# chinaxuyongtao/x264-vs2008

Hardware: AMD Instinct MI355X
Metric: encoded frames/sec, 1080p, preset=medium's flag set with the encoder's own lookahead and rate control (--crf 23 --b-adapt 1, hex, subme 7 RD, trellis 1, psy-rd, aq-mode 1, CABAC payload on the GPU); 1/2/4/8 MI355X (bit-exact) (higher is better)
Workload: dtype u8

## Files before the change

### x264_vs2008_amd/csrc/me_exact.h

```cpp
#pragma once
#include "device_prims.h"

#define MX_COST_MAX (1 << 28)
#define MX_COST_LDS 256

static __constant__ int c_subpel_iters[10][4] = {{0,0,0,0},{1,1,0,0},{0,1,1,0},{0,2,1,0},{0,2,1,1},{0,2,1,2},{0,0,2,2},{0,0,2,2},{0,0,4,10},{0,0,4,10}};

#define MX_GLB(T_) const __attribute__((address_space(1))) T_ *
#define MX_LDS(T_) const __attribute__((address_space(3))) T_ *
#define MX_UNI(v_) __builtin_amdgcn_readfirstlane(v_)

#define MX_NIB8(a, b, c_, d, e, f, g, h) ((u32)(((a) & 15) | (((b) & 15) << 4) | (((c_) & 15) << 8) | (((d) & 15) << 12) | (((e) & 15) << 16) | \
                                                (((f) & 15) << 20) | (((g) & 15) << 24) | (((u32)(h) & 15u) << 28)))
__device__ __forceinline__ int mx_nib(u32 pk, int i) { return ((int)(pk << (28 - 4 * i))) >> 28; }
#define MX_HEX2_DX MX_NIB8(-1, -2, -1, 1, 2, 1, -1, -2)
#define MX_HEX2_DY MX_NIB8(-2, 0, 2, 2, 0, -2, -2, 0)
#define MX_DIA_DX MX_NIB8(0, 0, -1, 1, 0, 0, 0, 0)
#define MX_DIA_DY MX_NIB8(-1, 1, 0, 0, 0, 0, 0, 0)

__device__ __forceinline__ void load16u(MX_GLB(u8) p, u32 o[4])
{
    const uintptr_t a = (uintptr_t)p;
    const u32 s = (u32)(a & 3);
    MX_GLB(u32) q = (MX_GLB(u32))(a - s);
// ... 707 lines not shown
            bdir = -1;
            for (int i = qpel; i > 0; i--) {
                const int ox = bx, oyy = by;
                odir = bdir;
                const int x = ox + mx_nib(MX_DIA_DX, g16), y = oyy + mx_nib(MX_DIA_DY, g16);
                const int cost = subpel_sum16_lane(c, x, y, satd, o.chroma_me) + c.lane_cost(x, y);
                const u32 key = mx_best_key<4>(cost, (g16 ^ 1) != odir, lane);
                if ((key >> 3) < (u32)bc) { bdir = (int)(key & 7u); MX_TAKE(4, key, bc, x, y, bx, by); }
                if (bx == ox && by == oyy) break;
            }
            if (by > L.smax1) {
                by = L.smax1;
                bc = __builtin_amdgcn_readlane(subpel_sum16_lane(c, bx, by, satd, o.chroma_me), 0) + c.cost(bx, by);
            }
            out_cost_mv = c.cost(bx, by);
        }
        mvx = bx; mvy = by; mcost = bc;
    } else if (mvy > L.smax1) mvy = L.smax1;
#undef INRANGE
    out_mvx = mvx; out_mvy = mvy;
    return mcost;
}

__device__ __forceinline__ int me_refine_qpel16(const MxCtx &c_in, const MeLimits &L_in, const MeOpts &o_in, int cost_in, int &mvx, int &mvy)
{
    MxCtx c = mx_uniform(c_in);
    c.patch_on = false;
    const MeLimits L = mx_uniform(L_in);
    const MeOpts o = mx_uniform(o_in);
    const int lane = c.lane, g16 = lane >> 4;
    const int hpel = c_subpel_iters[o.subme][0], qpel = c_subpel_iters[o.subme][1], satd = o.subme > 1 && !o.sad_only;
    int bx = MX_UNI(mvx), by = MX_UNI(mvy), bc = MX_UNI(cost_in);
    if (c.has_patch) mx_load_patch(c, bx, by);
    if (hpel && o.subme < 3) {
        const int mx = clip3(c.mvpx, L.smin0, L.smax0), my = clip3(c.mvpy, L.smin1, L.smax1);
        if ((mx - bx) | (my - by)) {
            const int cst = __builtin_amdgcn_readlane(sad_qpel16_lane(c, mx, my), 0) + c.cost(mx, my);
            if (cst < bc) { bc = cst; bx = mx; by = my; }
        }
    }
    for (int i = hpel; i > 0; i--) {
        const int ox = bx, oyy = by;
        const int x = ox + 2 * mx_nib(MX_DIA_DX, g16), y = oyy + 2 * mx_nib(MX_DIA_DY, g16);
        const int cost = sad_qpel16_lane(c, x, y) + c.lane_cost(x, y);
        const u32 key = mx_best_key<4>(cost, true, lane);
        MX_TAKE(4, key, bc, x, y, bx, by);
        if (bx == ox && by == oyy) break;
    }
    for (int i = qpel; i > 0; i--) {
        const int ox = bx, oyy = by;
        const int x = ox + mx_nib(MX_DIA_DX, g16), y = oyy + mx_nib(MX_DIA_DY, g16);
        const int cost = subpel_sum16_lane(c, x, y, satd, o.chroma_me) + c.lane_cost(x, y);
        const u32 key = mx_best_key<4>(cost, true, lane);
        MX_TAKE(4, key, bc, x, y, bx, by);
        if (bx == ox && by == oyy) break;
    }
    if (by > L.smax1) {
        by = L.smax1;
        bc = __builtin_amdgcn_readlane(subpel_sum16_lane(c, bx, by, satd, o.chroma_me), 0) + c.cost(bx, by);
    }
    mvx = bx; mvy = by;
    return bc;
}

__device__ __forceinline__ u32 mr_row_min16(u32 v)
{
    v = min(v, (u32)dpp_mov<0x128>((int)v)); v = min(v, (u32)dpp_mov<0x124>((int)v));
    v = min(v, (u32)dpp_mov<0x122>((int)v)); v = min(v, (u32)dpp_mov<0x121>((int)v));
    return v;
}
__device__ __forceinline__ int mr_from(int v, int src) { return __builtin_amdgcn_ds_bpermute(src << 2, v); }
__device__ __forceinline__ MX_GLB(u8) mr_plane(uint64_t plv, int sb, int k)
{
    const u32 lo = (u32)mr_from((int)(u32)plv, sb + k), hi = (u32)mr_from((int)(u32)(plv >> 32), sb + k);
    return (MX_GLB(u8))(((uint64_t)hi << 32) | lo);
}
__device__ __forceinline__ int mr_cost(const MxCtx &c, int qx, int qy, int mvpx, int mvpy)
{
    const int dx = qx - mvpx, dy = qy - mvpy;
    const bool in = c.has_cost_l && (unsigned)(dx + MX_COST_LDS) <= 2u * MX_COST_LDS && (unsigned)(dy + MX_COST_LDS) <= 2u * MX_COST_LDS;
    if (__ballot(!in) == 0) return (int)c.cost_l[dx + MX_COST_LDS] + (int)c.cost_l[dy + MX_COST_LDS];
    return (int)c.cost_g[dx] + (int)c.cost_g[dy];
}
template <int NR> __device__ __forceinline__ int mr_sad_rows(const MxCtx &c, uint64_t plv, int sb, int qx, int qy, int row0)
{
    const int fx = qx & 3, fy = qy & 3, idx = fy * 4 + fx;
    const ptrdiff_t base = (ptrdiff_t)((qy >> 2) + row0) * c.sy + (qx >> 2);
    MX_GLB(u8) pa = mr_plane(plv, sb, c_qpel_a[idx]) + base + (fy == 3) * c.sy;
    MX_GLB(u8) pb = mr_plane(plv, sb, c_qpel_b[idx]) + base + (fx == 3);
    u32 s = 0;
#pragma unroll
    for (int y = 0; y < NR; y++) {
        u32 a0, a1, t;
        load9u(pa + (ptrdiff_t)y * c.sy, a0, a1, t);
        if (idx & 5) { u32 b0, b1; load9u(pb + (ptrdiff_t)y * c.sy, b0, b1, t); a0 = avg4(a0, b0); a1 = avg4(a1, b1); }
        MX_LDS(u32) f = c.fe + c.fe_off + 4 * (row0 + y);
        s = sad4(a0, f[0], s); s = sad4(a1, f[1], s);
    }
    return (int)s;
}
__device__ __forceinline__ int mr_subpel_sum4(const MxCtx &c, uint64_t plv, int sb, int qx, int qy, int satd, int chroma, int u)
{
    int v = 0;
    u32 d[4][4];
    bool have_d = false;
    const int fx = qx & 3, fy = qy & 3, idx = fy * 4 + fx;
    MX_GLB(u8) qa = mr_plane(plv, sb, u < 2 ? (int)c_qpel_a[idx] : u + 2);
    MX_GLB(u8) qb = mr_plane(plv, sb, c_qpel_b[idx]);
    if (u < 2) {
        const int by = 4 * u;
        const ptrdiff_t base = (ptrdiff_t)((qy >> 2) + by) * c.sy + (qx >> 2);
        MX_GLB(u8) pa = qa + base + (fy == 3) * c.sy;
        MX_GLB(u8) pb = qb + base + (fx == 3);
        u32 f[4][2], p[4][2];
#pragma unroll
        for (int y = 0; y < 4; y++) {
            u32 t;
            load9u(pa + (ptrdiff_t)y * c.sy, p[y][0], p[y][1], t);
            if (idx & 5) {
                u32 b0, b1;
                load9u(pb + (ptrdiff_t)y * c.sy, b0, b1, t);
                p[y][0] = avg4(p[y][0], b0); p[y][1] = avg4(p[y][1], b1);
            }
            f[y][0] = c.fe[c.fe_off + (by + y) * 4]; f[y][1] = c.fe[c.fe_off + (by + y) * 4 + 1];
        }
        if (satd) {
#pragma unroll
            for (int y = 0; y < 4; y++)
#pragma unroll
                for (int x = 0; x < 4; x++) d[y][x] = mx_pair(f[y][1], f[y][0], x) - mx_pair(p[y][1], p[y][0], x);
            have_d = true;
        } else v = blk8x4_cost(f, p, 0);
    } else if (chroma) {
        MX_GLB(u8) plane = qa;
        MX_LDS(u8) fe = (u == 2 ? c.fe_u : c.fe_v) + c.cfe_off;
        const int dx = qx & 7, dy = qy & 7;
        const int ca = (8 - dx) * (8 - dy), cb = dx * (8 - dy), cc = (8 - dx) * dy, cd = dx * dy;
        MX_GLB(u8) s = plane + (ptrdiff_t)(qy >> 3) * c.sc + (qx >> 3);
        u32 r0[5], r1[5], r2[5];
#pragma unroll
        for (int y = 0; y < 5; y++) load9u(s + (ptrdiff_t)y * c.sc, r0[y], r1[y], r2[y]);
        if (satd) {
            u32 a[5][5];
#pragma unroll
            for (int y = 0; y < 5; y++) {
#pragma unroll
                for (int x = 0; x < 4; x++) a[y][x] = mx_pair(r1[y], r0[y], x);
                a[y][4] = mx_pair(r2[y], r1[y], 0);
            }
            const mx_u16x2 ka = {(unsigned short)ca, (unsigned short)ca}, kb = {(unsigned short)cb, (unsigned short)cb};
            const mx_u16x2 kc = {(unsigned short)cc, (unsigned short)cc}, kd = {(unsigned short)cd, (unsigned short)cd}, k32 = {32, 32};
#pragma unroll
            for (int y = 0; y < 4; y++) {
                MX_LDS(u32) fr = (MX_LDS(u32))(fe + y * 8);
                const u32 f0 = fr[0], f1 = fr[1];
#pragma unroll
                for (int x = 0; x < 4; x++) {
                    const mx_u16x2 pv = (mx_as_pk(a[y][x]) * ka + mx_as_pk(a[y][x + 1]) * kb + mx_as_pk(a[y + 1][x]) * kc + mx_as_pk(a[y + 1][x + 1]) * kd + k32) >> 6;
                    d[y][x] = (mx_pair(f1, f0, x) & 0xffffu) - (mx_as_u32(pv) & 0xffffu);
                }
            }
            have_d = true;
        } else {
            u32 f[4][2], p[4][2];
#pragma unroll
            for (int y = 0; y < 4; y++) {
                u32 w0 = 0;
#pragma unroll
                for (int x = 0; x < 4; x++) {
                    const int a0 = byte_of(r0[y], x), a1 = x < 3 ? byte_of(r0[y], x + 1) : byte_of(r1[y], 0);
                    const int b0 = byte_of(r0[y + 1], x), b1 = x < 3 ? byte_of(r0[y + 1], x + 1) : byte_of(r1[y + 1], 0);
                    w0 |= (u32)((ca * a0 + cb * a1 + cc * b0 + cd * b1 + 32) >> 6) << (8 * x);
                }
                p[y][0] = w0; f[y][0] = ((MX_LDS(u32))(fe + y * 8))[0];
                p[y][1] = 0u; f[y][1] = 0u;
            }
            v = blk8x4_cost(f, p, 0);
        }
    }
    if (have_d) v = satd8x4_packed(d);
    return quad_sum4(v);
}

__device__ __forceinline__ int me_search_refs8(const MxCtx &c_in, uint64_t plv, const MeLimits &L_in, const MeOpts &o_in, MX_LDS(i16) mvc, int n_mvc,
                                               bool live, int mvpx, int mvpy, int &out_mvx, int &out_mvy, int &out_cost_mv)
{
    MxCtx c = c_in;
    c.cost_g = mx_uni_ptr(c_in.cost_g); c.sy = MX_UNI(c_in.sy); c.sc = MX_UNI(c_in.sc); c.fe_off = MX_UNI(c_in.fe_off); c.cfe_off = MX_UNI(c_in.cfe_off);
    const MeLimits L = mx_uniform(L_in);
    const MeOpts o = mx_uniform(o_in);
    n_mvc = MX_UNI(n_mvc);
    const int j = c.lane & 15, sb = c.lane & 48, k8 = j >> 1, k4 = j >> 2;
    const int satd = !o.sad_only;
#define INRANGE(x_, y_) ((x_) >= L.fmin0 && (x_) <= L.fmax0 && (y_) >= L.fmin1 && (y_) <= L.fmax1)
#define MR_KEY(SH_, cost_, ok_) mr_row_min16((ok_) ? ((u32)(cost_) << 3) | (u32)(j >> (SH_)) : 0xffffffffu)
#define MR_TAKE(SH_, key_, live_, bcost_, x_, y_, bx_, by_) do { const int l_ = sb + ((int)((key_) & 7u) << (SH_)); \
        const int tx_ = mr_from((x_), l_), ty_ = mr_from((y_), l_); \
        if ((live_) && ((key_) >> 3) < (u32)(bcost_)) { (bcost_) = (int)((key_) >> 3); (bx_) = tx_; (by_) = ty_; } } while (0)
    int bmx = clip3(mvpx, L.fmin0 * 4, L.fmax0 * 4), bmy = clip3(mvpy, L.fmin1 * 4, L.fmax1 * 4);
    int bcost = MX_COST_MAX, bpx = 0, bpy = 0, bpcost = MX_COST_MAX;
    {
        const int px = bmx, py = bmy;
        int x = px, y = py;
        bool ok = k8 == 0;
        if (k8 >= 1 && k8 <= n_mvc) {
            const int vx = (int)mvc[2 * (k8 - 1)], vy = (int)mvc[2 * (k8 - 1) + 1];
            if ((vx | vy) && (vx != (int)(i16)px || vy != (int)(i16)py)) {
                ok = true; x = clip3(vx, L.fmin0 * 4, L.fmax0 * 4); y = clip3(vy, L.fmin1 * 4, L.fmax1 * 4);
            }
        }
        int sad = mr_sad_rows<4>(c, plv, sb, x, y, 4 * (j & 1));
        sad += dpp_mov<DPP_XOR1>(sad);
        const u32 key = MR_KEY(1, sad + mr_cost(c, x, y, mvpx, mvpy), ok);
        MR_TAKE(1, key, true, bpcost, x, y, bpx, bpy);
    }
    bmx = (bpx + 2) >> 2; bmy = (bpy + 2) >> 2;
    {
        const int x = k8 == 0 ? bmx : 0, y = k8 == 0 ? bmy : 0;
        int sad = mr_sad_rows<4>(c, plv, sb, x << 2, y << 2, 4 * (j & 1));
        sad += dpp_mov<DPP_XOR1>(sad);
        const u32 key = MR_KEY(1, sad + mr_cost(c, x << 2, y << 2, mvpx, mvpy), k8 < 2);
        MR_TAKE(1, key, true, bcost, x, y, bmx, bmy);
    }
    {
        int dir = -2;
        {
            const int hi = (k8 < 6 ? k8 : 0) + 1;
            const int x = bmx + mx_nib(MX_HEX2_DX, hi), y = bmy + mx_nib(MX_HEX2_DY, hi);
            int sad = mr_sad_rows<4>(c, plv, sb, x << 2, y << 2, 4 * (j & 1));
            sad += dpp_mov<DPP_XOR1>(sad);
            const u32 key = MR_KEY(1, sad + mr_cost(c, x << 2, y << 2, mvpx, mvpy), k8 < 6);
            if ((key >> 3) < (u32)bcost) { bcost = (int)(key >> 3); dir = (int)(key & 7u); }
        }
        const int hex_steps = o.me_range / 2;
        bool go = dir != -2;
        if (go) { bmx += mx_nib(MX_HEX2_DX, dir + 1); bmy += mx_nib(MX_HEX2_DY, dir + 1); }
        int i = 1;
        go = go && i < hex_steps && INRANGE(bmx, bmy);
        while (__ballot(go && live)) {
            const int odir = dir + 1 >= 7 ? dir - 6 : dir + 1 <= 0 ? dir + 6 : dir;
            const int idx = odir + (k8 < 3 ? k8 : 0);
            const int x = bmx + mx_nib(MX_HEX2_DX, idx), y = bmy + mx_nib(MX_HEX2_DY, idx);
            int sad = mr_sad_rows<4>(c, plv, sb, x << 2, y << 2, 4 * (j & 1));
            sad += dpp_mov<DPP_XOR1>(sad);
            const u32 key = MR_KEY(1, sad + mr_cost(c, x << 2, y << 2, mvpx, mvpy), k8 < 3);
            if (go) {
                if ((key >> 3) >= (u32)bcost) go = false;
                else {
                    bcost = (int)(key >> 3); dir = odir - 1 + (int)(key & 7u);
                    bmx += mx_nib(MX_HEX2_DX, dir + 1); bmy += mx_nib(MX_HEX2_DY, dir + 1);
                    i++;
                    go = i < hex_steps && INRANGE(bmx, bmy);
                }
            }
        }
        const int x = bmx + mx_nib(MX_NIB8(0, 0, -1, 1, -1, -1, 1, 1), k8), y = bmy + mx_nib(MX_NIB8(-1, 1, 0, 0, -1, 1, -1, 1), k8);
        int sad = mr_sad_rows<4>(c, plv, sb, x << 2, y << 2, 4 * (j & 1));
        sad += dpp_mov<DPP_XOR1>(sad);
        const u32 key = MR_KEY(1, sad + mr_cost(c, x << 2, y << 2, mvpx, mvpy), true);
        MR_TAKE(1, key, true, bcost, x, y, bmx, bmy);
    }
    int bx, by, bc;
    if (bpcost < bcost) { bx = bpx; by = bpy; bc = bpcost; }
    else { bx = bmx << 2; by = bmy << 2; bc = bcost; }
    const int hpel = c_subpel_iters[o.subme][2], qpel = c_subpel_iters[o.subme][3];
    {
        bool go = hpel > 0;
        int it = hpel;
        while (__ballot(go && live)) {
            const int ox = bx, oy = by;
            const int x = ox + 2 * mx_nib(MX_DIA_DX, k4), y = oy + 2 * mx_nib(MX_DIA_DY, k4);
            const int sad = quad_sum4(mr_sad_rows<2>(c, plv, sb, x, y, 2 * (j & 3)));
            const u32 key = MR_KEY(2, sad + mr_cost(c, x, y, mvpx, mvpy), true);
            MR_TAKE(2, key, go, bc, x, y, bx, by);
            if (go) go = --it > 0 && (bx != ox || by != oy);
        }
    }
    if (by > L.smax1) by = L.smax1;
    bc = mr_subpel_sum4(c, plv, sb, bx, by, satd, o.chroma_me, j & 3) + mr_cost(c, bx, by, mvpx, mvpy);
    {
        int bdir = -1, it = qpel;
        bool go = qpel > 0;
        while (__ballot(go && live)) {
            const int ox = bx, oy = by, odir = bdir;
            const int x = ox + mx_nib(MX_DIA_DX, k4), y = oy + mx_nib(MX_DIA_DY, k4);
            const int cost = mr_subpel_sum4(c, plv, sb, x, y, satd, o.chroma_me, j & 3) + mr_cost(c, x, y, mvpx, mvpy);
            const u32 key = MR_KEY(2, cost, (k4 ^ 1) != odir);
            const bool win = go && (key >> 3) < (u32)bc;
            MR_TAKE(2, key, go, bc, x, y, bx, by);
            if (win) bdir = (int)(key & 7u);
            if (go) go = --it > 0 && (bx != ox || by != oy);
        }
    }
    const bool clamp = by > L.smax1;
    if (__ballot(clamp && live)) {
        if (clamp) by = L.smax1;
        const int cost = mr_subpel_sum4(c, plv, sb, bx, by, satd, o.chroma_me, j & 3) + mr_cost(c, bx, by, mvpx, mvpy);
        if (clamp) bc = cost;
    }
    out_cost_mv = mr_cost(c, bx, by, mvpx, mvpy);
#undef MR_TAKE
#undef MR_KEY
#undef INRANGE
    out_mvx = bx; out_mvy = by;
    return bc;
}
```

### x264_vs2008_amd/csrc/slice_sweep_body.h

```cpp
    static_assert(!CH || RD, "the chain table belongs to the raster variant");
    SwRd rd_l;
    if constexpr (CH) {
        typedef const __attribute__((address_space(4))) SwDesc *desc_p;
        const desc_p d = (desc_p)(uintptr_t)tab + blockIdx.x;
        typedef const __attribute__((address_space(4))) u32 *word_p;
        static_assert(sizeof(SwArgs) % 4 == 0 && sizeof(SwRd) % 4 == 0 && alignof(SwDesc) >= 4, "copied by dwords");
        const word_p wa = (word_p)&d->a, wr = (word_p)&d->r;
#pragma unroll
        for (unsigned i = 0; i < sizeof(SwArgs) / 4; i++) ((u32 *)&a)[i] = wa[i];
#pragma unroll
        for (unsigned i = 0; i < sizeof(SwRd) / 4; i++) ((u32 *)&rd_l)[i] = wr[i];
    }
    const SwRd &rd = CH ? rd_l : rd_k;
    const SwRefs &refs = CH ? tab[blockIdx.x].t : refs_k;
    if constexpr (CH && !BS) __builtin_amdgcn_s_setprio(3);
    static_assert(!BS || RD, "B slices run in the raster variant");
    static_assert(!TD || BS, "temporal direct prediction is a B-slice matter");
    static_assert(!RF || (RD && !BS), "the RD refinement is built for the raster variant's I / P kernel");
#undef IS_SKIP_T
#define IS_SKIP_T(t) (BS ? ((t) == T_P_SKIP || (t) == T_B_SKIP) : (t) == T_P_SKIP)
    __builtin_assume(a.lossless == (int)LL);
    __shared__ SwLds s;
    __shared__ typename std::conditional<BS, SwLdsRdB, typename std::conditional<RF, SwLdsRdF, typename std::conditional<RD, SwLdsRd, SwLdsNone>::type>::type>::type sr_;
    SwLdsRd &sr = *(SwLdsRd *)&sr_;
// ... 673 lines not shown
                    if (lane == 0) {
                        a.mvr[((size_t)r * nmb + mb) * 2] = (i16)smx; a.mvr[((size_t)r * nmb + mb) * 2 + 1] = (i16)smy;
                        s.left_mvr[r][0] = (i16)smx; s.left_mvr[r][1] = (i16)smy;
                        s.l0mvc[r][0][0] = (i16)smx; s.l0mvc[r][0][1] = (i16)smy;
                    }
                }
                if (early_skip) { type = T_P_SKIP; skip_mc = 1; }
                else {
                    type = T_P_L0;
                    auto aim = [&](int r, int w, int h, int bx, int by) {
#pragma unroll
                        for (int k = 0; k < 4; k++) c.pl[k] = (MX_GLB(u8))(refs.y[r][k] + by_ + oy + (ptrdiff_t)by * a.sy + bx);
                        c.cu = (MX_GLB(u8))(refs.u[r] + bc_ + oc + (ptrdiff_t)(by >> 1) * a.sc + (bx >> 1)); c.cv = (MX_GLB(u8))(refs.v[r] + bc_ + oc + (ptrdiff_t)(by >> 1) * a.sc + (bx >> 1));
                        c.set_block(w, h, bx, by);
                    };
                    auto pme_put = [&](int slot, int vx, int vy, int cost, int cost_mv, int r, int ref_cost, int px, int py) {
                        const int f = lane - slot * 8;
                        pme_v = f == 0 ? vx : f == 1 ? vy : f == 2 ? cost : f == 3 ? cost_mv : f == 4 ? r : f == 5 ? ref_cost : f == 6 ? px : f == 7 ? py : pme_v;
                    };
                    auto pme = [&](int slot, int f) -> int { return __builtin_amdgcn_readlane(pme_v, slot * 8 + f); };
                    auto cache_set = [&](int x, int y, int w, int h, int r, int vx, int vy, int set_mv) {
                        const int k = lane - 12, i = k & 7, j = k >> 3;
                        if (k >= 0 && i < 4 && j < 4 && i >= x && i < x + w && j >= y && j < y + h) {
                            cref_v = r;
                            if (set_mv) { cmvx_v = vx; cmvy_v = vy; }
                        }
                    };
                    auto predict_blk = [&](int cur_part, int idx, int width, int &px, int &py) {
                        const int i8 = mb_scan8_luma(idx), i_ref = __builtin_amdgcn_readlane(cref_v, i8);
                        int ra = __builtin_amdgcn_readlane(cref_v, i8 - 1), rb = __builtin_amdgcn_readlane(cref_v, i8 - 8), rc = __builtin_amdgcn_readlane(cref_v, i8 - 8 + width), kc = i8 - 8 + width;
                        if ((idx & 3) == 3 || (width == 2 && (idx & 3) == 2) || rc == -2) { kc = i8 - 8 - 1; rc = __builtin_amdgcn_readlane(cref_v, kc); }
                        const int ax = __builtin_amdgcn_readlane(cmvx_v, i8 - 1), ay = __builtin_amdgcn_readlane(cmvy_v, i8 - 1), bx = __builtin_amdgcn_readlane(cmvx_v, i8 - 8), byv = __builtin_amdgcn_readlane(cmvy_v, i8 - 8);
                        const int cx = __builtin_amdgcn_readlane(cmvx_v, kc), cy = __builtin_amdgcn_readlane(cmvy_v, kc);
                        if (cur_part == D_16x8) {
                            if (idx == 0 && rb == i_ref) { px = bx; py = byv; return; }
                            if (idx != 0 && ra == i_ref) { px = ax; py = ay; return; }
                        } else if (cur_part == D_8x16) {
                            if (idx == 0 && ra == i_ref) { px = ax; py = ay; return; }
                            if (idx != 0 && rc == i_ref) { px = cx; py = cy; return; }
                        }
                        const int cnt = (ra == i_ref) + (rb == i_ref) + (rc == i_ref);
                        if (cnt > 1) { px = mb_median(ax, bx, cx); py = mb_median(ay, byv, cy); }
                        else if (cnt == 1) { if (ra == i_ref) { px = ax; py = ay; } else if (rb == i_ref) { px = bx; py = byv; } else { px = cx; py = cy; } }
                        else if (rb == -2 && rc == -2 && ra != -2) { px = ax; py = ay; }
                        else { px = mb_median(ax, bx, cx); py = mb_median(ay, byv, cy); }
                    };
                    int i_cost = best;
                    int c8x8 = MX_COST_MAX, c16x8 = MX_COST_MAX, c8x16 = MX_COST_MAX;
                    auto search_partitions = [&]() {
                    part = D_16x16;
                    if (a.flags_inter & 0x10) {
                        cache_set(0, 0, 4, 4, ref, 0, 0, 0);
                        int cost8x8;
                        if (a.mixed_refs) {
                            int maxref = a.n_refs - 1;
                            const int tt = type_top == T_I_8x8 ? 0 : type_top, tl = left_type == T_I_8x8 ? 0 : left_type;
                            if (maxref > 0 && ref == 0 && tt && tl) {
                                maxref = 0;
                                maxref = max(maxref, __builtin_amdgcn_readlane(cref_v, 3)); maxref = max(maxref, __builtin_amdgcn_readlane(cref_v, 4)); maxref = max(maxref, __builtin_amdgcn_readlane(cref_v, 6));
                                maxref = max(maxref, __builtin_amdgcn_readlane(cref_v, 8)); maxref = max(maxref, __builtin_amdgcn_readlane(cref_v, 11)); maxref = max(maxref, __builtin_amdgcn_readlane(cref_v, 27));
                            }
                            bool multi = false;
                            if constexpr (RD && !BS) multi = maxref > 0 && mo.method == 1 && mo.subme >= 3;
                            for (int i = 0; i < 4; i++) {
                                int bcost = 0x7fffffff, bvx = 0, bvy = 0, bcm = 0, br = 0, bpx = 0, bpy = 0;
                                const int bx8 = 8 * (i & 1), by8 = 8 * (i >> 1);
                                for (int r0 = 0; multi && r0 <= maxref; r0 += 4) {
                                    const int nsl = min(maxref - r0 + 1, 4), slot = lane >> 4, j = lane & 15;
                                    int lpx = 0, lpy = 0;
                                    for (int t = 0; t < nsl; t++) {
                                        cache_set(2 * (i & 1), 2 * (i >> 1), 2, 2, r0 + t, 0, 0, 0);
                                        int px, py;
                                        predict_blk(13, 4 * i, 2, px, py);
                                        if (slot == t || (t == 0 && slot >= nsl)) { lpx = px; lpy = py; }
                                    }
                                    const bool live = slot < nsl;
                                    const int r = r0 + (live ? slot : 0);
                                    const u8 *pb = j < 4 ? refs.y[r][j & 3] : j == 4 ? refs.u[r] : refs.v[r];
                                    const uint64_t plv = j < 4 ? (uint64_t)(uintptr_t)(pb + by_ + oy + (ptrdiff_t)by8 * a.sy + bx8)
                                                               : (uint64_t)(uintptr_t)(pb + bc_ + oc + (ptrdiff_t)(by8 >> 1) * a.sc + (bx8 >> 1));
                                    c.set_block(8, 8, bx8, by8);
                                    int vx, vy, cm;
                                    LAUNDER(); c.lane = lane;
                                    const int cost = me_search_refs8(c, plv, L, mo, (MX_LDS(i16))&s.l0mvc[r][0][0], i + 1, live, lpx, lpy, vx, vy, cm);
                                    for (int t = 0; t < nsl; t++) {
                                        const int rt = r0 + t, ct = __builtin_amdgcn_readlane(cost, 16 * t) + (Q.lambda * refs.ref_bits[rt]);
                                        const int tvx = __builtin_amdgcn_readlane(vx, 16 * t), tvy = __builtin_amdgcn_readlane(vy, 16 * t);
                                        if (lane == 0) { s.l0mvc[rt][i + 1][0] = (i16)tvx; s.l0mvc[rt][i + 1][1] = (i16)tvy; }
                                        if (ct < bcost) {
                                            bcost = ct; bvx = tvx; bvy = tvy; bcm = __builtin_amdgcn_readlane(cm, 16 * t); br = rt;
                                            bpx = __builtin_amdgcn_readlane(lpx, 16 * t); bpy = __builtin_amdgcn_readlane(lpy, 16 * t);
                                        }
                                    }
                                    WAVE_SYNC();
                                }
                                for (int r = 0; !multi && r <= maxref; r++) {
                                    cache_set(2 * (i & 1), 2 * (i >> 1), 2, 2, r, 0, 0, 0);
                                    int px, py, vx, vy, cm;
                                    predict_blk(13, 4 * i, 2, px, py);
                                    aim(r, 8, 8, 8 * (i & 1), 8 * (i >> 1));
                                    c.mvpx = px; c.mvpy = py;
                                    LAUNDER(); c.lane = lane;
                                    int cost = me_search_ref16(c, L, mo, &s.l0mvc[r][0][0], i + 1, nullptr, vx, vy, cm) + (Q.lambda * refs.ref_bits[r]);
                                    if (lane == 0) { s.l0mvc[r][i + 1][0] = (i16)vx; s.l0mvc[r][i + 1][1] = (i16)vy; }
                                    WAVE_SYNC();
                                    if (cost < bcost) { bcost = cost; bvx = vx; bvy = vy; bcm = cm; br = r; bpx = px; bpy = py; }
                                }
                                cache_set(2 * (i & 1), 2 * (i >> 1), 2, 2, br, bvx, bvy, 1);
                                pme_put(i, bvx, bvy, bcost + Q.lambda, bcm, br, (Q.lambda * refs.ref_bits[br]), bpx, bpy);
                            }
                            cost8x8 = pme(0, 2) + pme(1, 2) + pme(2, 2) + pme(3, 2);
                            if (!a.cabac && !(pme(0, 4) | pme(1, 4) | pme(2, 4) | pme(3, 4))) cost8x8 -= (Q.lambda * refs.ref_bits[0]) * 4;
                        } else {
                            const int r = ref, ref_cost = a.cabac || r ? (Q.lambda * refs.ref_bits[r]) : 0;
                            if (lane == 0) { s.l0mvc[r][0][0] = (i16)mvx; s.l0mvc[r][0][1] = (i16)mvy; }
                            WAVE_SYNC();
                            for (int i = 0; i < 4; i++) {
                                int px, py, vx, vy, cm;
                                predict_blk(13, 4 * i, 2, px, py);
                                aim(r, 8, 8, 8 * (i & 1), 8 * (i >> 1));
                                c.mvpx = px; c.mvpy = py;
                                LAUNDER(); c.lane = lane;
                                const int cost = me_search_ref16(c, L, mo, &s.l0mvc[r][0][0], i + 1, nullptr, vx, vy, cm);
                                cache_set(2 * (i & 1), 2 * (i >> 1), 2, 2, r, vx, vy, 1);
                                if (lane == 0) { s.l0mvc[r][i + 1][0] = (i16)vx; s.l0mvc[r][i + 1][1] = (i16)vy; }
                                pme_put(i, vx, vy, cost + ref_cost + Q.lambda, cm, r, ref_cost, px, py);
                            }
                            cost8x8 = pme(0, 2) + pme(1, 2) + pme(2, 2) + pme(3, 2);
                            if (a.cabac) cost8x8 -= ref_cost;
                        }
                        if (cost8x8 < best) { type = T_P_8x8; part = D_8x8; i_cost = cost8x8; }
                        if ((a.flags_inter & 0x20) && type == T_P_8x8) {
                            MeOpts mo_sub = mo;
                            mo_sub.chroma_me = 0;
                            for (int i = 0; i < 4; i++) {
                                const int r = pme(i, 4), x0 = 2 * (i & 1), y0 = 2 * (i >> 1);
                                int c8 = 0, subt = D_L0_8x8;
                                for (int t = 0; t < 3; t++) {
                                    const int sw = t == 1 ? 2 : 1, sh = t == 2 ? 2 : 1, sn = t == 0 ? 4 : 2, rec0 = t == 0 ? 4 * i : t == 1 ? 16 + 2 * i : 24 + 2 * i;
                                    const int cvx = t == 0 ? pme(i, 0) : __builtin_amdgcn_readlane(sub_mx, 4 * i), cvy = t == 0 ? pme(i, 1) : __builtin_amdgcn_readlane(sub_my, 4 * i);
                                    int sum = 0;
                                    for (int k = 0; k < sn; k++) {
                                        const int x4 = x0 + (t == 0 ? (k & 1) : t == 2 ? k : 0), y4 = y0 + (t == 0 ? (k >> 1) : t == 1 ? k : 0);
                                        const int idx = 4 * i + (y4 - y0) * 2 + (x4 - x0);
                                        int px, py, vx, vy, cm;
                                        predict_blk(13, idx, sw, px, py);
                                        aim(r, 4 * sw, 4 * sh, 4 * x4, 4 * y4);
                                        c.mvpx = px; c.mvpy = py;
                                        WAVE_SYNC();
                                        if (lane < 2) s.mvc[0][lane] = (i16)(lane ? cvy : cvx);
                                        WAVE_SYNC();
                                        LAUNDER(); c.lane = lane;
                                        const int cost = me_search_ref16(c, L, mo_sub, &s.mvc[0][0], k == 0 ? 1 : 0, nullptr, vx, vy, cm);
                                        if (lane == rec0 + k) { sub_mx = vx; sub_my = vy; sub_cost = cost; sub_px = px; sub_py = py; }
                                        cache_set(x4, y4, sw, sh, r, vx, vy, 1);
                                        sum += cost;
                                    }
                                    int cst = sum + (Q.lambda * refs.ref_bits[r]) + Q.lambda * (t == 0 ? 5 : 3);
                                    if (a.chroma_me && a.subme >= 5) cst += sw_sub_chroma(s, refs, a, r, i, t, rec0, sub_mx, sub_my, satd, oc, bc_, lane);
                                    if (t == 0) {
                                        if (!(cst < pme(i, 2))) break;
                                        c8 = cst; subt = D_L0_4x4;
                                    } else if (cst < c8) { c8 = cst; subt = t; }
                                }
                                if (subt != D_L0_8x8) i_cost += c8 - pme(i, 2);
                                if (subt == D_L0_8x8) cache_set(x0, y0, 2, 2, r, pme(i, 0), pme(i, 1), 1);
                                else {
                                    const int sw = subt == D_L0_8x4 ? 2 : 1, sh = subt == D_L0_4x8 ? 2 : 1, sn = subt == D_L0_4x4 ? 4 : 2, rec0 = subt == D_L0_4x4 ? 4 * i : subt == D_L0_8x4 ? 16 + 2 * i : 24 + 2 * i;
                                    for (int k = 0; k < sn; k++)
                                        cache_set(x0 + (subt == D_L0_4x4 ? (k & 1) : subt == D_L0_4x8 ? k : 0), y0 + (subt == D_L0_4x4 ? (k >> 1) : subt == D_L0_8x4 ? k : 0), sw, sh, r,
                                                  __builtin_amdgcn_readlane(sub_mx, rec0 + k), __builtin_amdgcn_readlane(sub_my, rec0 + k), 1);
                                }
                                if (lane == i) sub_t = subt;
                            }
                            cost8x8 = i_cost;
                        }
                        const int thresh16x8 = pme(1, 3) + pme(2, 3);
                        if (cost8x8 < best + thresh16x8)
                            for (int dir = 0; dir < 2; dir++) {
                                int sum = 0;
                                for (int i = 0; i < 2; i++) {
                                    const int ra = dir ? pme(i, 4) : pme(2 * i, 4), rb = dir ? pme(i + 2, 4) : pme(2 * i + 1, 4), nr = ra == rb ? 1 : 2;
                                    int bcost = 0x7fffffff, bvx = 0, bvy = 0, bcm = 0, br = 0, bpx = 0, bpy = 0;
                                    for (int j = 0; j < nr; j++) {
                                        const int r = j ? rb : ra, k1 = dir ? i + 1 : 2 * i + 1, k2 = dir ? i + 3 : 2 * i + 2;
                                        WAVE_SYNC();
                                        if (lane < 6) {
                                            const int k = lane >> 1 == 0 ? 0 : lane >> 1 == 1 ? k1 : k2;
                                            s.mvc[lane >> 1][lane & 1] = s.l0mvc[r][k][lane & 1];
                                        }
                                        if (dir) cache_set(2 * i, 0, 2, 4, r, 0, 0, 0); else cache_set(0, 2 * i, 4, 2, r, 0, 0, 0);
                                        int px, py, vx, vy, cm;
                                        predict_blk(dir ? D_8x16 : D_16x8, dir ? 4 * i : 8 * i, dir ? 2 : 4, px, py);
                                        aim(r, dir ? 8 : 16, dir ? 16 : 8, dir ? 8 * i : 0, dir ? 0 : 8 * i);
                                        c.mvpx = px; c.mvpy = py;
                                        LAUNDER(); c.lane = lane;
                                        const int cost = me_search_ref16(c, L, mo, &s.mvc[0][0], 3, nullptr, vx, vy, cm) + (Q.lambda * refs.ref_bits[r]);
                                        if (cost < bcost) { bcost = cost; bvx = vx; bvy = vy; bcm = cm; br = r; bpx = px; bpy = py; }
                                    }
                                    if (dir) cache_set(2 * i, 0, 2, 4, br, bvx, bvy, 1); else cache_set(0, 2 * i, 4, 2, br, bvx, bvy, 1);
                                    pme_put(4 + 2 * dir + i, bvx, bvy, bcost, bcm, br, (Q.lambda * refs.ref_bits[br]), bpx, bpy);
                                    sum += bcost;
                                }
                                if (dir) c8x16 = sum; else c16x8 = sum;
                                if (sum < i_cost) { i_cost = sum; type = T_P_L0; part = dir ? D_8x16 : D_16x8; }
                            }
                        c8x8 = cost8x8;
                    }
                    };
                    auto refine_winner = [&]() {
                    if (part == D_16x16) {
                        aim(ref, 16, 16, 0, 0);
                        c.mvpx = bmvpx; c.mvpy = bmvpy;
                        best -= (Q.lambda * refs.ref_bits[ref]);
                        LAUNDER(); c.lane = lane;
                        best = me_refine_qpel16(c, L, mo, best, mvx, mvy);
                        i_cost = best;
                        if (lane < 16) { s.mv4[lane][0] = (i16)mvx; s.mv4[lane][1] = (i16)mvy; }
                        if (lane < 4) s.ref8[lane] = (signed char)ref;
                    } else {
                        i_cost = 0;
                        const int nblk = part == D_8x8 ? 4 : 2, slot0 = part == D_8x8 ? 0 : part == D_16x8 ? 4 : 6;
                        for (int i = 0; i < nblk; i++) {
                            const int subt = part == D_8x8 ? __builtin_amdgcn_readlane(sub_t, i) : D_L0_8x8, nj = subt == D_L0_8x8 ? 1 : subt == D_L0_4x4 ? 4 : 2;
                            for (int k = 0; k < nj; k++) {
                                int bx = part == D_8x8 ? 8 * (i & 1) : part == D_8x16 ? 8 * i : 0, by = part == D_8x8 ? 8 * (i >> 1) : part == D_16x8 ? 8 * i : 0;
                                int w = part == D_16x8 ? 16 : 8, h = part == D_8x16 ? 16 : 8;
                                const int r = pme(slot0 + i, 4);
                                int vx = pme(slot0 + i, 0), vy = pme(slot0 + i, 1), cin = pme(slot0 + i, 2) - pme(slot0 + i, 5);
                                MeOpts mo_r = mo;
                                c.mvpx = pme(slot0 + i, 6); c.mvpy = pme(slot0 + i, 7);
                                if (subt != D_L0_8x8) {
                                    const int rec = (subt == D_L0_4x4 ? 4 * i : subt == D_L0_8x4 ? 16 + 2 * i : 24 + 2 * i) + k;
                                    bx += 4 * (subt == D_L0_4x4 ? (k & 1) : subt == D_L0_4x8 ? k : 0); by += 4 * (subt == D_L0_4x4 ? (k >> 1) : subt == D_L0_8x4 ? k : 0);
                                    w = subt == D_L0_8x4 ? 8 : 4; h = subt == D_L0_4x8 ? 8 : 4;
                                    vx = __builtin_amdgcn_readlane(sub_mx, rec); vy = __builtin_amdgcn_readlane(sub_my, rec); cin = __builtin_amdgcn_readlane(sub_cost, rec);
                                    c.mvpx = __builtin_amdgcn_readlane(sub_px, rec); c.mvpy = __builtin_amdgcn_readlane(sub_py, rec);
                                    mo_r.chroma_me = 0;
                                }
                                aim(r, w, h, bx, by);
                                LAUNDER(); c.lane = lane;
                                i_cost += me_refine_qpel16(c, L, mo_r, cin, vx, vy);
                                WAVE_SYNC();
                                if (lane < 16) {
                                    const int x4 = (lane & 3) * 4, y4 = (lane >> 2) * 4;
                                    if (x4 >= bx && x4 < bx + w && y4 >= by && y4 < by + h) { s.mv4[lane][0] = (i16)vx; s.mv4[lane][1] = (i16)vy; }
                                }
                                if (lane < 4) {
                                    const int x8 = (lane & 1) * 8, y8 = (lane >> 1) * 8;
                                    if (x8 >= (bx & ~7) && x8 < (bx & ~7) + (w < 8 ? 8 : w) && y8 >= (by & ~7) && y8 < (by & ~7) + (h < 8 ? 8 : h)) s.ref8[lane] = (signed char)r;
                                }
                            }
                        }
                    }
                    };
                    if constexpr (!RD) {
                    search_partitions();
                    refine_winner();
                    WAVE_SYNC();
                    if (part == D_8x8) sub_t_mb = sub_t;
                    PROF(2);
// ... 397 lines not shown
```

Baseline: 466.3.

## Batch 16x8 and 8x16 partition searches across wave quarters with 128-pixel ME

Adds a 128-pixel variant of the wave-parallel ME search so that 16x8 and 8x16 half-partition searches, with both candidate refs, run together in one wave. Each 16-lane quarter handles one partition family and ref instead of looping serially over direction and ref. Chroma subpel cost is folded into the same lanes via per-lane candidate MVs. The intent is to cut serial ME passes and wave underuse for rectangular partitions, at the cost of more complex indexing and a risk to bit-exactness in the ordering of MVP and cache_set.

```diff
diff --git a/x264_vs2008_amd/csrc/me_exact.h b/x264_vs2008_amd/csrc/me_exact.h
--- a/x264_vs2008_amd/csrc/me_exact.h
+++ b/x264_vs2008_amd/csrc/me_exact.h
@@ -813,34 +813,43 @@
     if (__ballot(!in) == 0) return (int)c.cost_l[dx + MX_COST_LDS] + (int)c.cost_l[dy + MX_COST_LDS];
     return (int)c.cost_g[dx] + (int)c.cost_g[dy];
 }
-template <int NR> __device__ __forceinline__ int mr_sad_rows(const MxCtx &c, uint64_t plv, int sb, int qx, int qy, int row0)
+template <int NR> __device__ __forceinline__ int mr_sad_rows(const MxCtx &c, uint64_t plv, int sb, int qx, int qy, int seg0, bool wide)
 {
     const int fx = qx & 3, fy = qy & 3, idx = fy * 4 + fx;
+    const int row0 = wide ? seg0 >> 1 : seg0;
     const ptrdiff_t base = (ptrdiff_t)((qy >> 2) + row0) * c.sy + (qx >> 2);
     MX_GLB(u8) pa = mr_plane(plv, sb, c_qpel_a[idx]) + base + (fy == 3) * c.sy;
     MX_GLB(u8) pb = mr_plane(plv, sb, c_qpel_b[idx]) + base + (fx == 3);
     u32 s = 0;
 #pragma unroll
     for (int y = 0; y < NR; y++) {
+        const int dr = wide ? y >> 1 : y, xo = wide ? 8 * (y & 1) : 0;
+        const ptrdiff_t o = (ptrdiff_t)dr * c.sy + xo;
         u32 a0, a1, t;
-        load9u(pa + (ptrdiff_t)y * c.sy, a0, a1, t);
-        if (idx & 5) { u32 b0, b1; load9u(pb + (ptrdiff_t)y * c.sy, b0, b1, t); a0 = avg4(a0, b0); a1 = avg4(a1, b1); }
-        MX_LDS(u32) f = c.fe + c.fe_off + 4 * (row0 + y);
+        load9u(pa + o, a0, a1, t);
+        if (idx & 5) { u32 b0, b1; load9u(pb + o, b0, b1, t); a0 = avg4(a0, b0); a1 = avg4(a1, b1); }
+        MX_LDS(u32) f = c.fe + c.fe_off + 4 * (row0 + dr) + (xo >> 2);
         s = sad4(a0, f[0], s); s = sad4(a1, f[1], s);
     }
     return (int)s;
 }
-__device__ __forceinline__ int mr_subpel_sum4(const MxCtx &c, uint64_t plv, int sb, int qx, int qy, int satd, int chroma, int u)
-{
+template <int NPX> __device__ __forceinline__ int mr_subpel_sum4(const MxCtx &c, uint64_t plv, int sb, int qx, int qy, int satd, int chroma, int u, bool wide)
+{
+    const bool big = NPX == 128;
+    const bool do_l = big || u < 2, do_c = big ? !(wide && (u & 1)) : u >= 2;
+    const int lbx = big && wide ? 8 * (u & 1) : 0, lby = big && wide ? 4 * (u >> 1) : 4 * u;
+    const int cby = big && !wide ? 4 * (u & 1) : 0;
+    const bool cwide = big && wide;
     int v = 0;
     u32 d[4][4];
     bool have_d = false;
     const int fx = qx & 3, fy = qy & 3, idx = fy * 4 + fx;
-    MX_GLB(u8) qa = mr_plane(plv, sb, u < 2 ? (int)c_qpel_a[idx] : u + 2);
+    MX_GLB(u8) qa = mr_plane(plv, sb, big || u < 2 ? (int)c_qpel_a[idx] : u + 2);
     MX_GLB(u8) qb = mr_plane(plv, sb, c_qpel_b[idx]);
-    if (u < 2) {
-        const int by = 4 * u;
-        const ptrdiff_t base = (ptrdiff_t)((qy >> 2) + by) * c.sy + (qx >> 2);
+    MX_GLB(u8) qc = qa;
+    if constexpr (big) qc = mr_plane(plv, sb, 4 + (u >> 1));
+    if (do_l) {
+        const ptrdiff_t base = (ptrdiff_t)((qy >> 2) + lby) * c.sy + (qx >> 2) + lbx;
         MX_GLB(u8) pa = qa + base + (fy == 3) * c.sy;
         MX_GLB(u8) pb = qb + base + (fx == 3);
         u32 f[4][2], p[4][2];
@@ -853,7 +862,7 @@
                 load9u(pb + (ptrdiff_t)y * c.sy, b0, b1, t);
                 p[y][0] = avg4(p[y][0], b0); p[y][1] = avg4(p[y][1], b1);
             }
-            f[y][0] = c.fe[c.fe_off + (by + y) * 4]; f[y][1] = c.fe[c.fe_off + (by + y) * 4 + 1];
+            f[y][0] = c.fe[c.fe_off + (lby + y) * 4 + (lbx >> 2)]; f[y][1] = c.fe[c.fe_off + (lby + y) * 4 + (lbx >> 2) + 1];
         }
         if (satd) {
 #pragma unroll
@@ -862,12 +871,17 @@
                 for (int x = 0; x < 4; x++) d[y][x] = mx_pair(f[y][1], f[y][0], x) - mx_pair(p[y][1], p[y][0], x);
             have_d = true;
         } else v = blk8x4_cost(f, p, 0);
-    } else if (chroma) {
-        MX_GLB(u8) plane = qa;
-        MX_LDS(u8) fe = (u == 2 ? c.fe_u : c.fe_v) + c.cfe_off;
+    }
+    if constexpr (big) {
+        if (have_d) v = satd8x4_packed(d);
+        have_d = false;
+    }
+    if (do_c && chroma) {
+        MX_GLB(u8) plane = qc;
+        MX_LDS(u8) fe = ((big ? u < 2 : u == 2) ? c.fe_u : c.fe_v) + c.cfe_off;
         const int dx = qx & 7, dy = qy & 7;
         const int ca = (8 - dx) * (8 - dy), cb = dx * (8 - dy), cc = (8 - dx) * dy, cd = dx * dy;
-        MX_GLB(u8) s = plane + (ptrdiff_t)(qy >> 3) * c.sc + (qx >> 3);
+        MX_GLB(u8) s = plane + (ptrdiff_t)((qy >> 3) + cby) * c.sc + (qx >> 3);
         u32 r0[5], r1[5], r2[5];
 #pragma unroll
         for (int y = 0; y < 5; y++) load9u(s + (ptrdiff_t)y * c.sc, r0[y], r1[y], r2[y]);
@@ -881,14 +895,15 @@
             }
             const mx_u16x2 ka = {(unsigned short)ca, (unsigned short)ca}, kb = {(unsigned short)cb, (unsigned short)cb};
             const mx_u16x2 kc = {(unsigned short)cc, (unsigned short)cc}, kd = {(unsigned short)cd, (unsigned short)cd}, k32 = {32, 32};
+            const u32 keep = cwide ? 0xffffffffu : 0x0000ffffu;
 #pragma unroll
             for (int y = 0; y < 4; y++) {
-                MX_LDS(u32) fr = (MX_LDS(u32))(fe + y * 8);
+                MX_LDS(u32) fr = (MX_LDS(u32))(fe + (cby + y) * 8);
                 const u32 f0 = fr[0], f1 = fr[1];
 #pragma unroll
                 for (int x = 0; x < 4; x++) {
                     const mx_u16x2 pv = (mx_as_pk(a[y][x]) * ka + mx_as_pk(a[y][x + 1]) * kb + mx_as_pk(a[y + 1][x]) * kc + mx_as_pk(a[y + 1][x + 1]) * kd + k32) >> 6;
-                    d[y][x] = (mx_pair(f1, f0, x) & 0xffffu) - (mx_as_u32(pv) & 0xffffu);
+                    d[y][x] = (mx_pair(f1, f0, x) & keep) - (mx_as_u32(pv) & keep);
                 }
             }
             have_d = true;
@@ -896,28 +911,34 @@
             u32 f[4][2], p[4][2];
 #pragma unroll
             for (int y = 0; y < 4; y++) {
-                u32 w0 = 0;
-#pragma unroll
-                for (int x = 0; x < 4; x++) {
-                    const int a0 = byte_of(r0[y], x), a1 = x < 3 ? byte_of(r0[y], x + 1) : byte_of(r1[y], 0);
-                    const int b0 = byte_of(r0[y + 1], x), b1 = x < 3 ? byte_of(r0[y + 1], x + 1) : byte_of(r1[y + 1], 0);
-                    w0 |= (u32)((ca * a0 + cb * a1 + cc * b0 + cd * b1 + 32) >> 6) << (8 * x);
+                u32 w0 = 0, w1 = 0;
+#pragma unroll
+                for (int x = 0; x < 8; x++) {
+                    const int a0 = x < 4 ? byte_of(r0[y], x) : byte_of(r1[y], x - 4), a1 = x < 3 ? byte_of(r0[y], x + 1) : x < 7 ? byte_of(r1[y], x - 3) : byte_of(r2[y], 0);
+                    const int b0 = x < 4 ? byte_of(r0[y + 1], x) : byte_of(r1[y + 1], x - 4), b1 = x < 3 ? byte_of(r0[y + 1], x + 1) : x < 7 ? byte_of(r1[y + 1], x - 3) : byte_of(r2[y + 1], 0);
+                    const u32 px = (u32)((ca * a0 + cb * a1 + cc * b0 + cd * b1 + 32) >> 6);
+                    if (x < 4) w0 |= px << (8 * x); else w1 |= px << (8 * (x - 4));
                 }
-                p[y][0] = w0; f[y][0] = ((MX_LDS(u32))(fe + y * 8))[0];
-                p[y][1] = 0u; f[y][1] = 0u;
-            }
-            v = blk8x4_cost(f, p, 0);
-        }
-    }
-    if (have_d) v = satd8x4_packed(d);
+                MX_LDS(u32) fr = (MX_LDS(u32))(fe + (cby + y) * 8);
+                p[y][0] = w0; f[y][0] = fr[0];
+                p[y][1] = cwide ? w1 : 0u; f[y][1] = cwide ? fr[1] : 0u;
+            }
+            v += blk8x4_cost(f, p, 0);
+        }
+    }
+    if (have_d) v += satd8x4_packed(d);
     return quad_sum4(v);
 }
 
-__device__ __forceinline__ int me_search_refs8(const MxCtx &c_in, uint64_t plv, const MeLimits &L_in, const MeOpts &o_in, MX_LDS(i16) mvc, int n_mvc,
+template <int NPX = 64>
+__device__ __forceinline__ int me_search_refs8(const MxCtx &c_in, uint64_t plv, const MeLimits &L_in, const MeOpts &o_in, int cvx, int cvy, int n_mvc,
                                                bool live, int mvpx, int mvpy, int &out_mvx, int &out_mvy, int &out_cost_mv)
 {
     MxCtx c = c_in;
-    c.cost_g = mx_uni_ptr(c_in.cost_g); c.sy = MX_UNI(c_in.sy); c.sc = MX_UNI(c_in.sc); c.fe_off = MX_UNI(c_in.fe_off); c.cfe_off = MX_UNI(c_in.cfe_off);
+    c.cost_g = mx_uni_ptr(c_in.cost_g); c.sy = MX_UNI(c_in.sy); c.sc = MX_UNI(c_in.sc);
+    if constexpr (NPX == 64) { c.fe_off = MX_UNI(c_in.fe_off); c.cfe_off = MX_UNI(c_in.cfe_off); }
+    const bool wide = NPX == 128 && c.bw == 16;
+    constexpr int NF = NPX / 16, NH = NPX / 32;
     const MeLimits L = mx_uniform(L_in);
     const MeOpts o = mx_uniform(o_in);
     n_mvc = MX_UNI(n_mvc);
@@ -935,12 +956,12 @@
         int x = px, y = py;
         bool ok = k8 == 0;
         if (k8 >= 1 && k8 <= n_mvc) {
-            const int vx = (int)mvc[2 * (k8 - 1)], vy = (int)mvc[2 * (k8 - 1) + 1];
+            const int vx = cvx, vy = cvy;
             if ((vx | vy) && (vx != (int)(i16)px || vy != (int)(i16)py)) {
                 ok = true; x = clip3(vx, L.fmin0 * 4, L.fmax0 * 4); y = clip3(vy, L.fmin1 * 4, L.fmax1 * 4);
             }
         }
-        int sad = mr_sad_rows<4>(c, plv, sb, x, y, 4 * (j & 1));
+        int sad = mr_sad_rows<NF>(c, plv, sb, x, y, NF * (j & 1), wide);
         sad += dpp_mov<DPP_XOR1>(sad);
         const u32 key = MR_KEY(1, sad + mr_cost(c, x, y, mvpx, mvpy), ok);
         MR_TAKE(1, key, true, bpcost, x, y, bpx, bpy);
@@ -948,7 +969,7 @@
     bmx = (bpx + 2) >> 2; bmy = (bpy + 2) >> 2;
     {
         const int x = k8 == 0 ? bmx : 0, y = k8 == 0 ? bmy : 0;
-        int sad = mr_sad_rows<4>(c, plv, sb, x << 2, y << 2, 4 * (j & 1));
+        int sad = mr_sad_rows<NF>(c, plv, sb, x << 2, y << 2, NF * (j & 1), wide);
         sad += dpp_mov<DPP_XOR1>(sad);
         const u32 key = MR_KEY(1, sad + mr_cost(c, x << 2, y << 2, mvpx, mvpy), k8 < 2);
         MR_TAKE(1, key, true, bcost, x, y, bmx, bmy);
@@ -958,7 +979,7 @@
         {
             const int hi = (k8 < 6 ? k8 : 0) + 1;
             const int x = bmx + mx_nib(MX_HEX2_DX, hi), y = bmy + mx_nib(MX_HEX2_DY, hi);
-            int sad = mr_sad_rows<4>(c, plv, sb, x << 2, y << 2, 4 * (j & 1));
+            int sad = mr_sad_rows<NF>(c, plv, sb, x << 2, y << 2, NF * (j & 1), wide);
             sad += dpp_mov<DPP_XOR1>(sad);
             const u32 key = MR_KEY(1, sad + mr_cost(c, x << 2, y << 2, mvpx, mvpy), k8 < 6);
             if ((key >> 3) < (u32)bcost) { bcost = (int)(key >> 3); dir = (int)(key & 7u); }
@@ -972,7 +993,7 @@
             const int odir = dir + 1 >= 7 ? dir - 6 : dir + 1 <= 0 ? dir + 6 : dir;
             const int idx = odir + (k8 < 3 ? k8 : 0);
             const int x = bmx + mx_nib(MX_HEX2_DX, idx), y = bmy + mx_nib(MX_HEX2_DY, idx);
-            int sad = mr_sad_rows<4>(c, plv, sb, x << 2, y << 2, 4 * (j & 1));
+            int sad = mr_sad_rows<NF>(c, plv, sb, x << 2, y << 2, NF * (j & 1), wide);
             sad += dpp_mov<DPP_XOR1>(sad);
             const u32 key = MR_KEY(1, sad + mr_cost(c, x << 2, y << 2, mvpx, mvpy), k8 < 3);
             if (go) {
@@ -986,7 +1007,7 @@
             }
         }
         const int x = bmx + mx_nib(MX_NIB8(0, 0, -1, 1, -1, -1, 1, 1), k8), y = bmy + mx_nib(MX_NIB8(-1, 1, 0, 0, -1, 1, -1, 1), k8);
-        int sad = mr_sad_rows<4>(c, plv, sb, x << 2, y << 2, 4 * (j & 1));
+        int sad = mr_sad_rows<NF>(c, plv, sb, x << 2, y << 2, NF * (j & 1), wide);
         sad += dpp_mov<DPP_XOR1>(sad);
         const u32 key = MR_KEY(1, sad + mr_cost(c, x << 2, y << 2, mvpx, mvpy), true);
         MR_TAKE(1, key, true, bcost, x, y, bmx, bmy);
@@ -1001,21 +1022,21 @@
         while (__ballot(go && live)) {
             const int ox = bx, oy = by;
             const int x = ox + 2 * mx_nib(MX_DIA_DX, k4), y = oy + 2 * mx_nib(MX_DIA_DY, k4);
-            const int sad = quad_sum4(mr_sad_rows<2>(c, plv, sb, x, y, 2 * (j & 3)));
+            const int sad = quad_sum4(mr_sad_rows<NH>(c, plv, sb, x, y, NH * (j & 3), wide));
             const u32 key = MR_KEY(2, sad + mr_cost(c, x, y, mvpx, mvpy), true);
             MR_TAKE(2, key, go, bc, x, y, bx, by);
             if (go) go = --it > 0 && (bx != ox || by != oy);
         }
     }
     if (by > L.smax1) by = L.smax1;
-    bc = mr_subpel_sum4(c, plv, sb, bx, by, satd, o.chroma_me, j & 3) + mr_cost(c, bx, by, mvpx, mvpy);
+    bc = mr_subpel_sum4<NPX>(c, plv, sb, bx, by, satd, o.chroma_me, j & 3, wide) + mr_cost(c, bx, by, mvpx, mvpy);
     {
         int bdir = -1, it = qpel;
         bool go = qpel > 0;
         while (__ballot(go && live)) {
             const int ox = bx, oy = by, odir = bdir;
             const int x = ox + mx_nib(MX_DIA_DX, k4), y = oy + mx_nib(MX_DIA_DY, k4);
-            const int cost = mr_subpel_sum4(c, plv, sb, x, y, satd, o.chroma_me, j & 3) + mr_cost(c, x, y, mvpx, mvpy);
+            const int cost = mr_subpel_sum4<NPX>(c, plv, sb, x, y, satd, o.chroma_me, j & 3, wide) + mr_cost(c, x, y, mvpx, mvpy);
             const u32 key = MR_KEY(2, cost, (k4 ^ 1) != odir);
             const bool win = go && (key >> 3) < (u32)bc;
             MR_TAKE(2, key, go, bc, x, y, bx, by);
@@ -1026,7 +1047,7 @@
     const bool clamp = by > L.smax1;
     if (__ballot(clamp && live)) {
         if (clamp) by = L.smax1;
-        const int cost = mr_subpel_sum4(c, plv, sb, bx, by, satd, o.chroma_me, j & 3) + mr_cost(c, bx, by, mvpx, mvpy);
+        const int cost = mr_subpel_sum4<NPX>(c, plv, sb, bx, by, satd, o.chroma_me, j & 3, wide) + mr_cost(c, bx, by, mvpx, mvpy);
         if (clamp) bc = cost;
     }
     out_cost_mv = mr_cost(c, bx, by, mvpx, mvpy);
diff --git a/x264_vs2008_amd/csrc/slice_sweep_body.h b/x264_vs2008_amd/csrc/slice_sweep_body.h
--- a/x264_vs2008_amd/csrc/slice_sweep_body.h
+++ b/x264_vs2008_amd/csrc/slice_sweep_body.h
@@ -779,7 +779,8 @@
                                     c.set_block(8, 8, bx8, by8);
                                     int vx, vy, cm;
                                     LAUNDER(); c.lane = lane;
-                                    const int cost = me_search_refs8(c, plv, L, mo, (MX_LDS(i16))&s.l0mvc[r][0][0], i + 1, live, lpx, lpy, vx, vy, cm);
+                                    const int kc = min(max((j >> 1) - 1, 0), i);
+                                    const int cost = me_search_refs8(c, plv, L, mo, s.l0mvc[r][kc][0], s.l0mvc[r][kc][1], i + 1, live, lpx, lpy, vx, vy, cm);
                                     for (int t = 0; t < nsl; t++) {
                                         const int rt = r0 + t, ct = __builtin_amdgcn_readlane(cost, 16 * t) + (Q.lambda * refs.ref_bits[rt]);
                                         const int tvx = __builtin_amdgcn_readlane(vx, 16 * t), tvy = __builtin_amdgcn_readlane(vy, 16 * t);
@@ -873,7 +874,57 @@
                             cost8x8 = i_cost;
                         }
                         const int thresh16x8 = pme(1, 3) + pme(2, 3);
-                        if (cost8x8 < best + thresh16x8)
+                        bool halves = false;
+                        if constexpr (RD && !BS) halves = mo.method == 1 && mo.subme >= 3;
+                        if (cost8x8 < best + thresh16x8 && halves) {
+                            const int sl = lane >> 4, j = lane & 15, fam = sl >> 1;
+                            int sum16x8 = 0, sum8x16 = 0;
+                            for (int i = 0; i < 2; i++) {
+                                int lpx = 0, lpy = 0, lr = 0;
+                                bool live = false;
+                                for (int d = 0; d < 2; d++) {
+                                    const int ra = d ? pme(i, 4) : pme(2 * i, 4), rb = d ? pme(i + 2, 4) : pme(2 * i + 1, 4), nr = ra == rb ? 1 : 2;
+                                    if (i) { if (d) cache_set(0, 0, 2, 4, pme(6, 4), pme(6, 0), pme(6, 1), 1); else cache_set(0, 0, 4, 2, pme(4, 4), pme(4, 0), pme(4, 1), 1); }
+                                    for (int t = 0; t < nr; t++) {
+                                        const int r = t ? rb : ra;
+                                        if (d) cache_set(2 * i, 0, 2, 4, r, 0, 0, 0); else cache_set(0, 2 * i, 4, 2, r, 0, 0, 0);
+                                        int px, py;
+                                        predict_blk(d ? D_8x16 : D_16x8, d ? 4 * i : 8 * i, d ? 2 : 4, px, py);
+                                        if (fam == d && (t == 0 || (sl & 1))) { lpx = px; lpy = py; lr = r; }
+                                    }
+                                    if (fam == d) live = (sl & 1) < nr;
+                                }
+                                const int bx = fam ? 8 * i : 0, by = fam ? 0 : 8 * i;
+                                const u8 *pb = j < 4 ? refs.y[lr][j & 3] : j == 4 ? refs.u[lr] : refs.v[lr];
+                                const uint64_t plv = j < 4 ? (uint64_t)(uintptr_t)(pb + by_ + oy + (ptrdiff_t)by * a.sy + bx)
+                                                           : (uint64_t)(uintptr_t)(pb + bc_ + oc + (ptrdiff_t)(by >> 1) * a.sc + (bx >> 1));
+                                const int k8 = j >> 1, kc = k8 <= 1 ? 0 : k8 == 2 ? (fam ? i + 1 : 2 * i + 1) : (fam ? i + 3 : 2 * i + 2);
+                                WAVE_SYNC();
+                                const int cvx = s.l0mvc[lr][kc][0], cvy = s.l0mvc[lr][kc][1];
+                                MxCtx ch = c;
+                                ch.set_block(fam ? 8 : 16, fam ? 16 : 8, bx, by);
+                                int vx, vy, cm;
+                                LAUNDER(); ch.lane = lane;
+                                const int cost = me_search_refs8<128>(ch, plv, L, mo, cvx, cvy, 3, live, lpx, lpy, vx, vy, cm);
+                                for (int d = 0; d < 2; d++) {
+                                    const int ra = d ? pme(i, 4) : pme(2 * i, 4), rb = d ? pme(i + 2, 4) : pme(2 * i + 1, 4), nr = ra == rb ? 1 : 2;
+                                    int bcost = 0x7fffffff, bvx = 0, bvy = 0, bcm = 0, br = 0, bpx = 0, bpy = 0;
+                                    for (int t = 0; t < nr; t++) {
+                                        const int r = t ? rb : ra, l0 = 16 * (2 * d + t), ct = __builtin_amdgcn_readlane(cost, l0) + (Q.lambda * refs.ref_bits[r]);
+                                        if (ct < bcost) {
+                                            bcost = ct; bvx = __builtin_amdgcn_readlane(vx, l0); bvy = __builtin_amdgcn_readlane(vy, l0); bcm = __builtin_amdgcn_readlane(cm, l0); br = r;
+                                            bpx = __builtin_amdgcn_readlane(lpx, l0); bpy = __builtin_amdgcn_readlane(lpy, l0);
+                                        }
+                                    }
+                                    pme_put(4 + 2 * d + i, bvx, bvy, bcost, bcm, br, (Q.lambda * refs.ref_bits[br]), bpx, bpy);
+                                    if (d) sum8x16 += bcost; else sum16x8 += bcost;
+                                }
+                            }
+                            cache_set(2, 0, 2, 4, pme(7, 4), pme(7, 0), pme(7, 1), 1);
+                            c16x8 = sum16x8; c8x16 = sum8x16;
+                            if (c16x8 < i_cost) { i_cost = c16x8; type = T_P_L0; part = D_16x8; }
+                            if (c8x16 < i_cost) { i_cost = c8x16; type = T_P_L0; part = D_8x16; }
+                        } else if (cost8x8 < best + thresh16x8)
                             for (int dir = 0; dir < 2; dir++) {
                                 int sum = 0;
                                 for (int i = 0; i < 2; i++) {
```

Result: slower. 440.7 (-5.5%).
